# TigreGotico/phoonnx

Measured on AMD Instinct MI355X. Metric: audio samples/sec (22.05 kHz), batch-32 256-phoneme utterances, higher is better.
Workload: dtype f32 (f16x3 split: fp32 operands as two fp16 planes, three MFMA products, fp32 accumulate)

## Files before the change

### include/vitsmi.h

```cpp
#ifndef VITSMI_H
#define VITSMI_H

#include <stddef.h>
#include <stdint.h>

#ifdef __cplusplus
extern "C" {
#endif

typedef struct vits_handle vits_handle;

enum {
    VITS_OK = 0,
    VITS_E_IO = -1,
    VITS_E_FORMAT = -2,
    VITS_E_ARG = -3,
    VITS_E_DEVICE = -4,
    VITS_E_NOMEM = -5,
    VITS_E_RANGE = -6
};

#define VITS_MAX_DIMS 4


// ... 148 lines not shown
int vits_test_conv1d_sx(int device_id, const float *x, int B, int Cin, int T, const float *w, const float *bias,
                        int Cout, int K, int dil, int pad_l, int flags, float slope, float *out);
int vits_test_conv1d_sx_planar(int device_id, const float *x, int B, int Cin, int T, const float *w, const float *bias,
                               int Cout, int K, int dil, int flags, const int64_t *lens, const float *old, int row_split,
                               int pl_rows, float *out, float *planes_out);
long long vits_test_set_sx_small_max(long long wgs);
int vits_test_conv1d_sx_gate(int device_id, const float *x, int B, int Cin, int T, const float *w, const float *bias,
                             const float *bias_b, int Cout, int K, int dil, int flags, float *out);
int vits_test_conv_transpose1d_sx(int device_id, const float *x, int B, int Cin, int T, const float *w,
                                  const float *bias, int Cout, int K, int stride, float *out);
int vits_bench_conv1d_sx(int device_id, int B, int Cin, int Cout, int T, int K, int dil, int dbg, int iters,
                         float *ms_out);
int vits_test_conv_pair_sx(int device_id, const float *x, int B, int C, int T, const float *w1, const float *b1,
                           const float *w2, const float *b2, int K, int dil1, int dil2, int chain, float slope, float *out,
                           float *ms_out);
int vits_test_attention(int device_id, const float *qkv, int B, int C, int T, int n_heads, const float *rel_k,
                        const float *rel_v, int window, const int64_t *lens, float *out);
int vits_test_attention16(int device_id, const float *qkv, int B, int C, int T, int n_heads, const float *rel_k,
                          const float *rel_v, int window, const int64_t *lens, float *out, uint16_t *out_planes, int kernel,
                          int reps, float *ms_out);

int vits_test_resample(int device_id, const float *x, const int64_t *lens, int B, int S, int in_rate, int out_rate, float *y,
                       int64_t S_out);
int vits_test_resample_pieces(int device_id, const float *x, const int64_t *lens, int B, int S, int in_rate, int out_rate,
                              int piece_samples, float *y, int64_t S_out, int64_t *ranges, int max_ranges);

int vits_test_durations(int device_id, const float *logw, const int64_t *dur, const int64_t *lens, int B, int T, float length_scale,
                        const float *rows, const float *token_rate, float *w_ceil, int32_t *cum, int32_t *y_len);
int vits_test_expand_prior(int device_id, const float *m_logs, int B, int C, int T, const int32_t *cum, const int64_t *lens,
                           const int32_t *y_len, int F, const float *noise, int64_t noise_stride, int noise_frames,
// ... 12 lines not shown
```

### phoonnx_amd/_ffi.py

```python
import ctypes as C
import os

import numpy as np

_HERE = os.path.dirname(os.path.abspath(__file__))
_LIB = None

VITS_MAX_DIMS = 4


class VitsNoise(C.Structure):
    _fields_ = [("noise_dp", C.c_void_p), ("noise_z", C.c_void_p), ("noise_z_stride", C.c_int64),
                ("seed", C.c_uint64)]


class VitsOutput(C.Structure):
    _fields_ = [("data", C.POINTER(C.c_float)), ("dims", C.c_int64 * 4), ("y_lengths", C.POINTER(C.c_int64))]


class VitsStats(C.Structure):
    _fields_ = [("conv_flops", C.c_double), ("conv_bytes", C.c_double), ("dec_flops", C.c_double),
                ("dec_bytes", C.c_double), ("flow_flops", C.c_double), ("enc_flops", C.c_double),
                ("dp_flops", C.c_double), ("conv_ms", C.c_float), ("dec_ms", C.c_float), ("flow_ms", C.c_float),
                ("enc_ms", C.c_float), ("dp_ms", C.c_float), ("total_ms", C.c_float), ("conv_launches", C.c_int),
# ... 18 lines not shown

CHUNK_FN = C.CFUNCTYPE(C.c_int, C.c_void_p, C.POINTER(C.c_float), C.c_int, C.c_int64, C.c_int64, C.c_int64)

VITS_E_RANGE = -6


EXPORTS = [
    "vits_open", "vits_open_with_arena", "vits_open_host", "vits_open_layout", "vits_open_opts", "vits_close",
    "vits_run_chunked", "vits_run_vocoder_chunked", "vits_last_error", "vits_num_inputs",
    "vits_input_name", "vits_meta", "vits_hparam", "vits_arena_bytes", "vits_arena_host", "vits_arena_device",
    "vits_run", "vits_free_output", "vits_run_device", "vits_sync", "vits_last_y_lengths", "vits_last_pcm16", "vits_run_vocoder",
    "vits_tap",
    "vits_set_timing", "vits_set_tails", "vits_reserve", "vits_get_stats", "vits_stream", "vits_test_conv1d", "vits_test_conv_transpose1d",
    "vits_test_attention", "vits_test_attention16", "vits_bench_conv1d", "vits_test_conv1d_sx", "vits_test_conv1d_sx_planar", "vits_test_conv1d_sx_gate", "vits_test_set_sx_small_max",
    "vits_test_conv_transpose1d_sx",
    "vits_bench_conv1d_sx", "vits_test_conv_pair_sx", "vits_fetch_output", "vits_run_async", "vits_host_alloc", "vits_host_free",
    "vits_launch_records", "vits_run_async_rows", "vits_run_device_rows", "vits_run_chunked_rows",
    "vits_run_async_ctl", "vits_run_chunked_ctl", "vits_last_durations",
    "vits_set_output_rate", "vits_last_sample_counts", "vits_resample_plan", "vits_test_resample", "vits_test_resample_pieces",
    "vits_test_durations", "vits_test_expand_prior", "vits_test_fill_normal", "vits_test_fill_normal_rows", "vits_test_post_conv",
]


G2P_EXPORTS = ["g2p_open", "g2p_close", "g2p_last_error", "g2p_hparam", "g2p_num_outputs", "g2p_output_name", "g2p_bucket",
               "g2p_run", "g2p_generate", "g2p_generate_batch", "g2p_test_forced_steps", "g2p_test_linear", "g2p_test_step"]


def lib_path():
    return os.environ.get("VITSMI_LIB") or os.path.join(_HERE, "libvitsmi.so")


# ... 82 lines not shown
                                               C.c_int, vp]
    lib.vits_test_attention.argtypes = [C.c_int, vp, C.c_int, C.c_int, C.c_int, C.c_int, vp, vp, C.c_int, vp, vp]
    lib.vits_test_attention16.argtypes = [C.c_int, vp, C.c_int, C.c_int, C.c_int, C.c_int, vp, vp, C.c_int, vp, vp, vp,
                                          C.c_int, C.c_int, f32p]
    lib.vits_bench_conv1d.argtypes = [C.c_int] * 11 + [f32p]
    lib.vits_test_conv1d_sx.argtypes = lib.vits_test_conv1d.argtypes
    lib.vits_test_conv_transpose1d_sx.argtypes = lib.vits_test_conv_transpose1d.argtypes
    lib.vits_test_conv1d_sx_planar.argtypes = [C.c_int, vp, C.c_int, C.c_int, C.c_int, vp, vp, C.c_int, C.c_int, C.c_int, C.c_int,
                                               vp, vp, C.c_int, C.c_int, vp, vp]
    lib.vits_test_set_sx_small_max.argtypes = [C.c_longlong]
    lib.vits_test_set_sx_small_max.restype = C.c_longlong
    lib.vits_test_conv1d_sx_gate.argtypes = [C.c_int, vp, C.c_int, C.c_int, C.c_int, vp, vp, vp, C.c_int, C.c_int, C.c_int, C.c_int, vp]
    lib.vits_bench_conv1d_sx.argtypes = [C.c_int] * 9 + [f32p]
    lib.vits_test_conv_pair_sx.argtypes = [C.c_int, vp, C.c_int, C.c_int, C.c_int, vp, vp, vp, vp, C.c_int, C.c_int,
                                           C.c_int, C.c_int, C.c_float, vp, f32p]
    lib.g2p_open.argtypes = [C.c_char_p, C.c_int, C.POINTER(vp)]
    lib.g2p_close.argtypes = [vp]
    lib.g2p_close.restype = None
    lib.g2p_last_error.argtypes = [vp]
    lib.g2p_last_error.restype = C.c_char_p
    lib.g2p_hparam.argtypes = [vp, C.c_char_p, i64p]
    lib.g2p_num_outputs.argtypes = [vp]
    lib.g2p_output_name.argtypes = [vp, C.c_int]
    lib.g2p_output_name.restype = C.c_char_p
    lib.g2p_bucket.argtypes = [vp, C.c_int, C.c_int]
    lib.g2p_run.argtypes = [vp, vp, C.c_int, vp, vp, C.c_int, vp]
    lib.g2p_generate.argtypes = [vp, vp, C.c_int, C.c_int, C.c_int64, C.c_int64, vp, C.POINTER(C.c_int)]
    lib.g2p_generate_batch.argtypes = [vp, vp, vp, C.c_int, C.c_int, C.c_int64, C.c_int64, vp, vp]
    lib.g2p_test_forced_steps.argtypes = [vp, vp, vp, C.c_int, vp, C.c_int, vp]
    lib.g2p_test_linear.argtypes = [C.c_int, C.c_int, vp, vp, C.c_int, vp, C.c_int, C.c_int, vp, C.c_int64, C.c_int64, C.c_int, vp]
# ... 12 lines not shown
```

### phoonnx_amd/csrc/conv_sx_pair.hip.hpp

```cpp
#pragma once
#include <cstdlib>
#include "conv_geom.hpp"
#include "conv_sx_engine.hip.hpp"

namespace vitsmi {

struct SxPairArgs {
    const float *xr;
    float islope, mslope;
    int T;
    const u32x4 *wp1, *wp2;
    const float *bias1, *bias2;
    float wscale1, wscale2;
    float *out_raw;
    const float *zeros;
    int C, nchunks;
    int K1, dil1, pad1;
    int K2, dil2, pad2;
    int LW1;
    unsigned x_bytes;
    int LW2;
    unsigned y_chunk_bytes;
    int BNo, NT, B;
    int flags;
// ... 35 lines not shown
#ifndef SX_PAIR_WGS32
#define SX_PAIR_WGS32 3
#endif
#ifndef SX_PAIR_EARLY32
#define SX_PAIR_EARLY32 1
#endif
#ifndef SX_PAIR_ST_SC1
#define SX_PAIR_ST_SC1 0
#endif
#ifndef SX_PAIR_ONE_READ64
#define SX_PAIR_ONE_READ64 1
#endif
#ifndef SX_PAIR_ONE_READ32
#define SX_PAIR_ONE_READ32 1
#endif
template <int MW, int NW, int WM, int WN, int EPI, bool CHAIN, int NCH = 1>
__global__ __launch_bounds__(256, (NW == 2 && !SX_PAIR_EARLY_ACC && NCH == 1) ? SX_PAIR_WGS32 : 2) void conv_sx_pair_kernel(SxPairArgs a) {
    constexpr int BN = NW * WN * 32, NH = NW / 2;
    static_assert(NCH == 1 || (CHAIN && NW == 2 && (EPI & EPI_ACC) == 0), "fused chains: 32 channels, no external running sum");
    constexpr bool ONE_READ = NW == 4 ? SX_PAIR_ONE_READ64 != 0 : SX_PAIR_ONE_READ32 != 0;
    constexpr bool EARLY = ONE_READ || (NW == 2 && SX_PAIR_EARLY32);
    constexpr int DEPTH = NW == 2 ? SX_PAIR_DEPTH32 : SX_PAIR_DEPTH64;
    static_assert(DEPTH >= 2 && DEPTH <= 6, "wait_a covers up to five younger sets");
    constexpr bool ACC = (EPI & EPI_ACC) != 0 && SX_PAIR_EARLY_ACC;
    static_assert(!(ONE_READ && ACC), "the running sum is not pulled into the single-read prologue");
    static_assert(WM * WN == 4 && MW == 1 && BN == 256, "one block row per wave, 256 columns");
    constexpr int NPW = 2, STEPBYTES = WM * MW * NPW * 1024;
    constexpr int MAXCH = WM * 2;
    extern __shared__ __attribute__((aligned(16))) unsigned char lds_sx[];
    const int tid = threadIdx.x, lane = tid & 63;
    const int wave = __builtin_amdgcn_readfirstlane(tid >> 6);
    const int wm = wave / WN, wn = wave % WN;
    const int l31 = lane & 31, hi = lane >> 5;
    const int wg_xcd = blockIdx.x & 7, wg_seq = blockIdx.x >> 3;
    const int tile_nb = __builtin_amdgcn_readfirstlane(sx_xcd_tile(wg_seq, wg_xcd, a.xgs));
    if (tile_nb >= a.NT * a.B) return;
    const int b = tile_nb / a.NT, t0 = (tile_nb - b * a.NT) * a.BNo;
    const int t1 = t0 - a.pad2;
    const int T = a.T, LW = a.LW1;
    const int TV = __builtin_amdgcn_readfirstlane(sx_valid_cols(a.rag, b, T));
    if (t0 >= TV) return;
    const uint32_t lds0 = (uint32_t)(uintptr_t)lds_sx;
    const uint32_t XB = a.x_bytes;
    const char *wbase1 = reinterpret_cast<const char *>(a.wp1) + wm * (MW * NPW * 1024);
    const char *wbase2 = reinterpret_cast<const char *>(a.wp2) + wm * (MW * NPW * 1024);
    const float *xrb = a.xr + (int64_t)b * a.C * T;
    float pk = 0.f;

    struct ASet {
        u32x4 fa[2];
    };
    const uint32_t voff0 = (uint32_t)lane * 16u;
    auto load_a = [&](ASet &f, const char *wb, int step) {
// ... 29 lines not shown
        asm volatile("s_memtime %0\n\ts_waitcnt lgkmcnt(0)" : "=s"(t)::"memory");
        __builtin_amdgcn_sched_barrier(0);
        return t;
    };
    unsigned long long tp[8];
    tp[0] = stamp();
#endif
    if constexpr (NW == 2 && WM == 1 && NCH == 1 && SX_PAIR_SHARED_A != 0)
        for (int g = 0; g < 3; g++)
            if (g < ((a.nchunks * a.K1) >> 1)) {
                const int sub = wave >> 1, pl = wave & 1;
                lds_dma<16>(wbase1 + (int64_t)(2 * g + sub) * STEPBYTES + pl * 1024 + lane * 16,
                            reinterpret_cast<float *>(lds_sx + a.a_ring + (unsigned)((g * 2 + sub) * 2048 + pl * 1024)));
            }
    constexpr bool BIAS_LDS = NCH == 1;
    if constexpr (BIAS_LDS) {
        if (wave == 0) {
            constexpr int CC = WM * 32;
            const int k = lane - (lane >= CC / 4 ? CC / 4 : 0);
            const float *bp = lane < CC / 4 ? a.bias1 : a.bias2;
            const void *src = (bp && lane < CC / 2) ? static_cast<const void *>(bp + 4 * k) : static_cast<const void *>(a.zeros + 4 * (lane & 31));
            lds_dma<16>(src, reinterpret_cast<float *>(lds_sx + a.bias_off));
        }
    }
    auto bias_from_lds = [&](int conv, f32x4 (&bq)[4]) __attribute__((always_inline)) {
        u32x4 t4[4];
#pragma unroll
        for (int q = 0; q < 4; q++)
            asm volatile("ds_read_b128 %0, %1" : "=v"(t4[q]) : "v"(lds0 + a.bias_off + (uint32_t)(conv * (WM * 32) + wm * 32 + 8 * q + 4 * hi) * 4u) : "memory");
        asm volatile("s_waitcnt lgkmcnt(0)" ::: "memory");
        __builtin_amdgcn_sched_barrier(0);
#pragma unroll
        for (int q = 0; q < 4; q++) bq[q] = __builtin_bit_cast(f32x4, t4[q]);
    };
    constexpr int NXC = 3;
    if constexpr (ONE_READ) {
        constexpr int NXH = MAXCH, NG = 2 * MAXCH;
        const int HW = LW - 256, pad1 = a.pad1;
        const int nhc = HW * NG, nxh = (nhc + 255) >> 8;
        u32x4 hst[NXH][2];
        bool hin[NXH], hok[NXH];
        uint32_t hlds[NXH];
        const float *hp[NXH];
#pragma unroll
// ... 303 lines not shown
        for (int g = 0; g < NG; g++) {
            step(fa0, fa1, 2 * g, false);
            step(fa1, fa0, 2 * g + 1, true);
        }
    };

    struct ChainPar {
        const char *wb1, *wb2;
        const float *bias1, *bias2;
        float ws1, ws2;
        int K1, dil1, K2, dil2;
        uint32_t xoff, yoff;
    };
    auto chain_par = [&](int ci) {
        ChainPar c;
        if constexpr (NCH == 1) {
            c = ChainPar{wbase1, wbase2, a.bias1, a.bias2, a.wscale1, a.wscale2, a.K1, a.dil1, a.K2, a.dil2, 0u, 0u};
        } else {
            const auto &h = a.ch[ci];
            c = ChainPar{reinterpret_cast<const char *>(h.wp1) + wm * (MW * NPW * 1024),
                         reinterpret_cast<const char *>(h.wp2) + wm * (MW * NPW * 1024),
                         h.bias1, h.bias2, h.wscale1, h.wscale2, h.K1, h.dil1, h.K2, h.dil2, (uint32_t)h.xoff, (uint32_t)h.yoff};
        }
        return c;
    };
    static_assert(NCH == 1 || EARLY, "fused chains keep x in registers from the prologue on");
    const uint32_t ylds = NCH > 1 ? lds0 + (uint32_t)a.nchunks * XB : lds0;
    f32x4 xkeep[NCH > 1 ? NW / 2 : 1][2][4], tot[NCH > 1 ? NW / 2 : 1][2][4];
#if SX_PAIR_ALIAS
    ASet f1s[DEPTH + 1];
    ASet(&f2s)[DEPTH + 1] = f1s;
#else
    ASet f1s[DEPTH + 1], f2s[DEPTH + 1];
#endif
#pragma unroll 1
    for (int ci = 0; ci < NCH; ci++) {
    const ChainPar cp = chain_par(ci);
    if constexpr (NCH > 1) {
        if (ci > 0) {
#pragma unroll
            for (int rr = 0; rr < NW / 2; rr++)
#pragma unroll
                for (int j = 0; j < 2; j++)
#pragma unroll
                    for (int q = 0; q < 4; q++) pre[rr][j][q] = xkeep[rr][j][q];
            zero_acc();
        }
    }
    if constexpr (!SHA) load_a(f1s[0], cp.wb1, 0);
    if (ci == 0) {
        asm volatile("s_waitcnt lgkmcnt(0)" ::: "memory");
#if SX_PAIR_PROF
// ... 24 lines not shown
    if constexpr (SHA) sha_prefetch(cp.wb2, cp.K2);
    {
        const float wsc = cp.ws1, msl = a.mslope;
        const float *biasp = cp.bias1 ? cp.bias1 : a.zeros;
        const int b_on = cp.bias1 ? 1 : 0;
        const uint32_t YC = a.y_chunk_bytes, LW2 = (uint32_t)a.LW2;
        const int row0 = wm * 32;
        f32x4 bq[4];
        if constexpr (BIAS_LDS) bias_from_lds(0, bq);
        else {
#pragma unroll
            for (int q = 0; q < 4; q++) bq[q] = *reinterpret_cast<const f32x4 *>(biasp + (row0 + 8 * q + 4 * hi) * b_on);
        }
#pragma unroll
        for (int n = 0; n < NW; n++) {
            const int col = (wn * NW + n) * 32 + l31;
            const int t = t1 + col;
            const bool live = t >= 0 && t < TV;
#pragma unroll
            for (int q = 0; q < 4; q++) {
                float o[4];
#pragma unroll
                for (int e = 0; e < 4; e++) {
                    float v = __builtin_fmaf(acc[n][4 * q + e], wsc, bq[q][e]);
                    if constexpr (CHAIN) {
                        if constexpr (NCH > 1) {
                            if (ci == 0) xkeep[n / 2][n % 2][q][e] = pre[n / 2][n % 2][q][e];
                        }
                        v += pre[n / 2][n % 2][q][e];
                        pre[n / 2][n % 2][q][e] = v;
                    }
                    o[e] = live ? fmaxf(v, v * msl) : 0.f;
                }
                unsigned wa[2], wb[2];
                split2h_pair_pk(o[0], o[1], wa[0], wa[1], pk);
                split2h_pair_pk(o[2], o[3], wb[0], wb[1], pk);
                const int g = 4 * wm + q;
                const uint32_t cell = ylds + (uint32_t)(g >> 1) * YC + ((uint32_t)(g & 1) * LW2 + (uint32_t)(col + a.pad2)) * 16u + 8u * hi;
                asm volatile("ds_write_b64 %0, %1" ::"v"(cell), "v"(u32x2{wa[0], wb[0]}) : "memory");
                asm volatile("ds_write_b64 %0, %1" ::"v"(cell + 2u * LW2 * 16u), "v"(u32x2{wa[1], wb[1]}) : "memory");
            }
            asm volatile("" : "+v"(pk));
        }
    }
    zero_acc();
    asm volatile("s_waitcnt lgkmcnt(0)" ::: "memory");
    __builtin_amdgcn_s_barrier();
    __builtin_amdgcn_sched_barrier(0);
#if SX_PAIR_PROF
    tp[5] = stamp();
#endif

    if constexpr (SHA)
        run_conv_sha(f2s[0], f2s[1], cp.wb2, cp.K2, cp.dil2, ylds + (uint32_t)(hi * a.LW2 + wn * (NW * 32) + l31 + (int)cp.yoff) * 16u,
                     a.y_chunk_bytes, (uint32_t)(2 * a.LW2) * 16u);
    else
        run_conv(f2s, cp.wb2, cp.K2, cp.dil2, ylds + (uint32_t)(hi * a.LW2 + wn * (NW * 32) + l31 + (int)cp.yoff) * 16u,
                 a.y_chunk_bytes, (uint32_t)(2 * a.LW2) * 16u);
#if SX_PAIR_PROF
    tp[6] = stamp();
#endif
    if constexpr (!CHAIN && !EARLY) load_pre();

    {
        constexpr int flags = EPI;
        float *rawb = a.out_raw + (int64_t)b * a.C * T;
        const float wsc = cp.ws2, rdiv = a.div;
        const float *biasp = cp.bias2 ? cp.bias2 : a.zeros;
        const int b_on = cp.bias2 ? 1 : 0;
        const int row0 = wm * 32;
        f32x4 bq[4];
        if constexpr (BIAS_LDS) bias_from_lds(1, bq);
        else {
#pragma unroll
            for (int q = 0; q < 4; q++) bq[q] = *reinterpret_cast<const f32x4 *>(biasp + (row0 + 8 * q + 4 * hi) * b_on);
        }
        static_for<NW / 2>([&](auto R) {
            constexpr int rr = decltype(R)::value;
            f32x4 adl[2][4];
            if constexpr ((flags & EPI_ACC) != 0 && !(EARLY && ACC)) {
#pragma unroll
                for (int j = 0; j < 2; j++) {
                    const int t = t1 + (wn * NW + rr * 2 + j) * 32 + l31;
                    const int tl = t < 0 ? 0 : (t < T ? t : T - 1);
#pragma unroll
                    for (int q = 0; q < 4; q++)
                        adl[j][q] = *reinterpret_cast<const f32x4 *>(rawb + ((int64_t)((row0 >> 3) + q) * T + tl) * 8 + 4 * hi);
                }
            }
#pragma unroll
            for (int j = 0; j < 2; j++) {
                const int n = rr * 2 + j;
                const int col = (wn * NW + n) * 32 + l31;
                const int t = t1 + col;
                const bool kept = !(col < a.pad2 || col >= a.pad2 + a.BNo || t >= TV);
                if constexpr (NCH == 1) {
                    if (!kept) continue;
                }
#pragma unroll
                for (int q = 0; q < 4; q++) {
                    f32x4 v;
#pragma unroll
                    for (int e = 0; e < 4; e++) v[e] = __builtin_fmaf(acc[n][4 * q + e], wsc, bq[q][e]);
                    v += pre[rr][j][q];
                    if constexpr (NCH > 1) {
                        if (ci > 0) v += tot[rr][j][q];
                        tot[rr][j][q] = v;
                        if (ci < NCH - 1 || !kept) continue;
                    }
                    if constexpr ((flags & EPI_ACC) != 0) {
                        if constexpr (EARLY && ACC) v += ad[rr][j][q];
                        else v += adl[j][q];
                    }
                    if constexpr ((flags & EPI_DIV) != 0) {
#pragma unroll
                        for (int e = 0; e < 4; e++) v[e] = v[e] / rdiv;
                    }
#if SX_PAIR_ST_SC1
                    {
                        float *sp = rawb + ((int64_t)((row0 >> 3) + q) * T + t) * 8 + 4 * hi;
                        const f32x4 sv = v;
                        asm volatile("global_store_dwordx4 %0, %1, off sc1" ::"v"(sp), "v"(sv) : "memory");
                    }
#else
                    *reinterpret_cast<f32x4 *>(rawb + ((int64_t)((row0 >> 3) + q) * T + t) * 8 + 4 * hi) = v;
#endif
                }
            }
        });
    }
    }
#if SX_PAIR_PROF
    asm volatile("s_waitcnt vmcnt(0)" ::: "memory");
    tp[7] = stamp();
    if (a.prof && tid == 0) {
        for (int i = 0; i < 7; i++) atomicAdd(a.prof + i, tp[i + 1] - tp[i]);
        atomicAdd(a.prof + 7, 1ull);
    }
#endif
    if (a.peak) sx_publish_peak(a.peak, (int)blockIdx.x, pk);
}

template <int MW, int NW, int WM, int WN, int EPI, bool CHAIN, int NCH = 1>
inline hipError_t launch_conv_sx_pair_k(const SxPairArgs &a, dim3 grid, size_t lds, hipStream_t stream) {
    static std::atomic<uint64_t> attr_done{0};
    auto kern = conv_sx_pair_kernel<MW, NW, WM, WN, EPI, CHAIN, NCH>;
    if (hipError_t e = sx_allow_big_lds(reinterpret_cast<const void *>(kern), attr_done); e != hipSuccess) return e;
    if (g_launch_name_on)
        snprintf(g_launch_name, sizeof g_launch_name, "conv_sx_pair_kernel<%d, %d, %d, %d, %d, %s, %d>", MW, NW, WM, WN, EPI,
                 CHAIN ? "true" : "false", NCH);
    kern<<<grid, 256, lds, stream>>>(a);
    return hipGetLastError();
}

inline bool sx_pair_supported(int C, int cfg, int K1, int dil1, int K2, int dil2) {
    if (K1 < 3 || K2 < 3 || dil1 < 1 || dil2 < 1) return false;
    if (!((C == 64 && cfg == 1) || (C == 32 && cfg == 2))) return false;
    const int LW1 = 256 + (K1 - 1) * dil1;
    if (2 * LW1 > kSxRawStageCells) return false;
    const int halo2 = (K2 - 1) * dil2;
    static const int keep_min = [] {
        const char *e = std::getenv("VITSMI_PAIR_MIN_KEEP");
        return e ? std::atoi(e) : 160;
    }();
    if (halo2 % 2 || 256 - halo2 < keep_min) return false;
// ... 53 lines not shown
    }
    if (cfg == 1) {
        if (chain) {
            SX_PAIR_CASES(1, 4, 2, 2, true)
        }
        SX_PAIR_CASES(1, 4, 2, 2, false)
    }
    if (chain) {
        SX_PAIR_CASES(1, 2, 1, 4, true)
    }
    SX_PAIR_CASES(1, 2, 1, 4, false)
#undef SX_PAIR_CASES
}
#endif

struct SxMrfGeom {
    int pad1, pad2, LW1, LW2;
    size_t lds;
};
inline bool sx_mrf_geom(int C, int n, const int *K1, const int *dil1, const int *K2, const int *dil2, SxMrfGeom *g) {
    if (C != 32 || n < 2 || n > 3) return false;
    int p1 = 0, p2 = 0;
    for (int i = 0; i < n; i++) {
        if (K1[i] < 3 || K2[i] < 3 || !(K1[i] & 1) || !(K2[i] & 1) || dil1[i] < 1 || dil2[i] < 1) return false;
        const int a1 = (K1[i] - 1) / 2 * dil1[i], a2 = (K2[i] - 1) / 2 * dil2[i];
        p1 = a1 > p1 ? a1 : p1;
        p2 = a2 > p2 ? a2 : p2;
    }
    const int LW1 = 256 + 2 * p1;
    if (2 * LW1 > kSxRawStageCells) return false;
// ... 54 lines not shown
```

### phoonnx_amd/csrc/vitsmi.hip

```cpp
#include <climits>
#include <hip/hip_runtime.h>

#include <cmath>
#include <cstdarg>
#include <chrono>
#include <cstdio>
#include <cstring>
#include <mutex>
#include <string>
#include <vector>

#include "../../include/vitsmi.h"
#include "conv_geom.hpp"
#include "conv_sx_engine.hip.hpp"
#include "conv_sx_pair.hip.hpp"
#include "conv_sx_pair16.hip.hpp"
#include "attention16.hip.hpp"
#include "conv_sx_small.hip.hpp"
#include "kernels.hip.hpp"
#include "model.hpp"
#include "resample.hip.hpp"
#include "test_dev.hip.hpp"
#include "workspace.hpp"

// ... 652 lines not shown
                    fprintf(stderr, "pairprof row %d wgs %llu:", r, hrows[r * 8 + 7]);
                    for (int i = 0; i < 7; i++) fprintf(stderr, " %.0f", (double)hrows[r * 8 + i] / (double)hrows[r * 8 + 7]);
                    fprintf(stderr, "\n");
                }
            hipMemset(rows, 0, sizeof hrows);
        }
    }
#endif
    const bool ev = conv_event_begin(c);
    c.note(launch_conv_sx_pair(a, c1.cfg, c.B, c.st, chain));
    const double wf = c.work_frac();
    const double fl = 2.0 * (c1.macs_per_t + c2.macs_per_t) * (double)T * c.B * wf;
    const double by = 4.0 * c.B * ((double)(c1.Cin + c1.Cout) * T + (double)(c2.Cin + c2.Cout) * T) * wf;
    const ConvDesc *const members[] = {&c1, &c2};
    fused_launch_end(c, ev, members, 2, c1, T, fl, by);
}

bool sx_pair16_ok(const vits_handle *h, const ConvDesc &c1, const ConvDesc &c2) {
    static const bool off = [] {
        const char *e = std::getenv("VITSMI_PAIR16");
        return (e && e[0] == '0') || std::getenv("VITSMI_SX_NO_PAIR") != nullptr;
    }();
    if (off || c1.Cin != c1.Cout || c2.Cin != c2.Cout || c1.Cin != c2.Cin || c1.ups != 1 || c2.ups != 1) return false;
    if (c1.padL * 2 != (c1.K - 1) * c1.dil || c2.padL * 2 != (c2.K - 1) * c2.dil) return false;
    const bool h1 = c1.h1 && c2.h1, f3 = c1.f16 && c2.f16 && c1.s16 && c2.s16 && !c1.rawin && !c2.rawin;
    if (!h1 && !f3) return false;
    if (c1.cfg != c2.cfg || c1.cfg != (c1.Cin == 64 ? 1 : 2)) return false;
    (void)h;
    return sx_pair16_plan(c1.Cin, h1 ? 1 : 2, c1.K, c1.dil, c2.K, c2.dil, nullptr) != 0;
}
// ... 712 lines not shown
            auto step_out = [&](int q) {
                StepOut w{EPI_RES, rpl ? nullptr : ra[q & 1], fr ? nullptr : raa[q & 1]};
                if (q == rbk.n - 1) {
                    w.flags |= mrf_flags(j, nk);
                    w.raw = xs_raw;
                    w.pl = nullptr;
                    if (j == nk - 1 && !last_stage && !fr) {
                        w.pl = xs_pl;
                        w.flags |= SX_NO_RAW_STORE;
                    }
                }
                return w;
            };
            const float *cur = y_raw;
            const uint16_t *cura = y_pl;
            for (int q = 0; q < rbk.n; q++) {
                StepOut w = step_out(q);
                if (rbk.type1 && fr && sx_pair_ok(h, rbk.c1[q], rbk.c2[q])) {
                    conv_sx_pair(c, rbk.c1[q], rbk.c2[q], cur, T, w.raw, w.flags, (float)nk, S);
                } else if (!rbk.type1 && fr && q + 1 < rbk.n && sx_pair_ok(h, rbk.c1[q], rbk.c1[q + 1])) {
                    w = step_out(++q);
                    conv_sx_pair(c, rbk.c1[q - 1], rbk.c1[q], cur, T, w.raw, w.flags, (float)nk, S, true);
                } else {
                    const void *in = fr ? static_cast<const void *>(cur) : static_cast<const void *>(cura);
                    SxOpt res = rbk.type1 || rpl ? act : lrelu;
                    res.div = (float)nk;
                    if (rpl) {
                        res.res_pl = cura;
                        res.res_slope = S;
                    } else
// ... 1699 lines not shown
    a.C = C;
    a.K1 = d1.K; a.dil1 = d1.dil; a.pad1 = d1.padL;
    a.K2 = d2.K; a.dil2 = d2.dil; a.pad2 = d2.padL;
    a.div = 1.f;
    auto go = [&] { return launch_conv_sx_pair(a, d1.cfg, B, nullptr, chain != 0); };
    TCHECK(go());
    TCHECK(hipDeviceSynchronize());
    if (ms_out) TCHECK(time_launches(10, go, ms_out));
    sx_unblock_kernel<<<dim3((T + 255) / 256, C / 8, B), 256>>>(draw, nullptr, dout, C, T, 1);
    TCHECK(hipGetLastError());
    TCHECK(hipDeviceSynchronize());
    TCHECK(download(out, dout, n));
    return VITS_OK;
}

int vits_bench_conv1d_sx(int device_id, int B, int Cin, int Cout, int T, int K, int dil, int dbg, int iters,
                         float *ms_out) {
    if (int rc = test_dev(device_id)) return rc;
    std::vector<float> w((size_t)Cout * Cin * K), x((size_t)B * Cin * T);
    bench_fill(w, x);
    ConvDesc d;
    std::vector<float> arena;
    TestPack o = sx_test_pack((dbg & 64) ? SxPack::F16X1 : ((dbg & 128) ? SxPack::F16X2 : SxPack::BF16X3));
    o.sx.no_s16 = (dbg & (1 | 2 | 16 | 256)) != 0;
    std::string e = pack_test_conv(w.data(), nullptr, Cin, Cout, K, dil, dil * (K - 1) / 2, 3, &d, &arena, o);
    if (!e.empty()) return fail(nullptr, VITS_E_ARG, "%s", e.c_str());
    const size_t nx = x.size(), no = (size_t)B * Cout * T;
    DevBufs D;
    float *dA = D.up(arena.data(), arena.size());
    float *dx = D.up(x.data(), nx);
// ... 389 lines not shown
```

### phoonnx_amd/session.py

```python
import ctypes as C
import time
from dataclasses import dataclass
from typing import Dict, List, Optional, Sequence

import numpy as np

from . import _ffi


class SessionError(RuntimeError):
    """Raised for every failure of the engine (onnxruntime raises its own
    InvalidArgument/RuntimeException at voice.py:374; callers there do not catch either)."""


class RangeError(SessionError):
    """VITS_E_RANGE: the f16x3 generator arithmetic met an activation beyond the range of its fp16 operand planes
    (|x| > 65504) or a non-finite value.  The engine reports this instead of returning clamped audio; `MiSession`
    (range_fallback=True, the default) then reopens the voice with the bf16x6 arithmetic (fp32 range) and repeats the
    call, so user code only sees this when the fallback is switched off or impossible (borrowed weight arena)."""


class _PinnedPool:

    def __init__(self, keep_bytes=2 << 30):
# ... 1077 lines not shown
        raise ValueError("both convs are C -> C with the same kernel size")
    b1 = None if b1 is None else np.ascontiguousarray(b1, np.float32)
    b2 = None if b2 is None else np.ascontiguousarray(b2, np.float32)
    out = np.empty_like(x)
    ms = C.c_float(0.0)
    rc = lib.vits_test_conv_pair_sx(device_id, _ffi.ptr(x), B, Cc, T, _ffi.ptr(w1), _ffi.ptr(b1), _ffi.ptr(w2),
                                    _ffi.ptr(b2), K, dil1, dil2,
                                    (1 if chain else 0) | ({"pair": 0, "pair16": 1, "pair16_f16": 2}[kernel] << 1) | (8 if from_plane else 0),
                                    float(slope), _ffi.ptr(out),
                                    C.byref(ms) if timed else None)
    if rc != 0:
        raise SessionError(_ffi.last_error(None))
    return (out, float(ms.value)) if timed else out


def bench_conv1d_sx(B, Cin, Cout, T, K, dil=1, dbg=0, iters=20, device_id=0):
    lib = _ffi.load()
    res = np.zeros(8, np.float32)
    rc = lib.vits_bench_conv1d_sx(device_id, B, Cin, Cout, T, K, dil, dbg, iters,
                                  res.ctypes.data_as(_ffi.C.POINTER(_ffi.C.c_float)))
    if rc != 0:
        raise SessionError(_ffi.last_error(None))
    if dbg & 16:
        return float(res[0]), int(res[1]), [float(v) for v in res[3:8]] + [float(res[2])]
    return float(res[0]), int(res[1])


def test_conv_transpose1d(x, w, bias, stride, device_id=0, sx=False):
    lib = _ffi.load()
    x = np.ascontiguousarray(x, np.float32)
# ... 205 lines not shown
```

Measured before the change: 142.1 million.

## Fuse all steps of a ResBlock1 into one conv-pair kernel launch

Adds an NSTEP template mode to the paired-conv kernel so the 2-3 dilated conv pairs of one HiFi-GAN ResBlock1 run inside a single launch. Intermediate residual sums stay in registers and in LDS as fp16 planes instead of round-tripping through global memory between steps. Each tile computes shrinking halo margins and keeps only the central columns. This removes per-step launches and activation reads and writes, at the cost of redundant halo compute and larger LDS per workgroup, which may lower occupancy. A test and benchmark entry point is added as well.

Measured after the change: 143.3 million (median of 6 runs). Within noise of the previous version (+0.9%).

```diff
diff --git a/include/vitsmi.h b/include/vitsmi.h
--- a/include/vitsmi.h
+++ b/include/vitsmi.h
@@ -186,6 +186,8 @@
 int vits_test_conv_pair_sx(int device_id, const float *x, int B, int C, int T, const float *w1, const float *b1,
                            const float *w2, const float *b2, int K, int dil1, int dil2, int chain, float slope, float *out,
                            float *ms_out);
+int vits_test_resblock1_sx(int device_id, const float *x, int B, int C, int T, const float *ws, const float *bs, int K, int nstep,
+                           const int *dils, float slope, const float *acc, float div, float *out, float *ms_out);
 int vits_test_attention(int device_id, const float *qkv, int B, int C, int T, int n_heads, const float *rel_k,
                         const float *rel_v, int window, const int64_t *lens, float *out);
 int vits_test_attention16(int device_id, const float *qkv, int B, int C, int T, int n_heads, const float *rel_k,
diff --git a/phoonnx_amd/_ffi.py b/phoonnx_amd/_ffi.py
--- a/phoonnx_amd/_ffi.py
+++ b/phoonnx_amd/_ffi.py
@@ -56,7 +56,7 @@
     "vits_set_timing", "vits_set_tails", "vits_reserve", "vits_get_stats", "vits_stream", "vits_test_conv1d", "vits_test_conv_transpose1d",
     "vits_test_attention", "vits_test_attention16", "vits_bench_conv1d", "vits_test_conv1d_sx", "vits_test_conv1d_sx_planar", "vits_test_conv1d_sx_gate", "vits_test_set_sx_small_max",
     "vits_test_conv_transpose1d_sx",
-    "vits_bench_conv1d_sx", "vits_test_conv_pair_sx", "vits_fetch_output", "vits_run_async", "vits_host_alloc", "vits_host_free",
+    "vits_bench_conv1d_sx", "vits_test_conv_pair_sx", "vits_test_resblock1_sx", "vits_fetch_output", "vits_run_async", "vits_host_alloc", "vits_host_free",
     "vits_launch_records", "vits_run_async_rows", "vits_run_device_rows", "vits_run_chunked_rows",
     "vits_run_async_ctl", "vits_run_chunked_ctl", "vits_last_durations",
     "vits_set_output_rate", "vits_last_sample_counts", "vits_resample_plan", "vits_test_resample", "vits_test_resample_pieces",
@@ -169,6 +169,8 @@
     lib.vits_bench_conv1d_sx.argtypes = [C.c_int] * 9 + [f32p]
     lib.vits_test_conv_pair_sx.argtypes = [C.c_int, vp, C.c_int, C.c_int, C.c_int, vp, vp, vp, vp, C.c_int, C.c_int,
                                            C.c_int, C.c_int, C.c_float, vp, f32p]
+    lib.vits_test_resblock1_sx.argtypes = [C.c_int, vp, C.c_int, C.c_int, C.c_int, vp, vp, C.c_int, C.c_int, vp, C.c_float, vp,
+                                           C.c_float, vp, f32p]
     lib.g2p_open.argtypes = [C.c_char_p, C.c_int, C.POINTER(vp)]
     lib.g2p_close.argtypes = [vp]
     lib.g2p_close.restype = None
diff --git a/phoonnx_amd/csrc/conv_sx_pair.hip.hpp b/phoonnx_amd/csrc/conv_sx_pair.hip.hpp
--- a/phoonnx_amd/csrc/conv_sx_pair.hip.hpp
+++ b/phoonnx_amd/csrc/conv_sx_pair.hip.hpp
@@ -73,10 +73,11 @@
 #ifndef SX_PAIR_ONE_READ32
 #define SX_PAIR_ONE_READ32 1
 #endif
-template <int MW, int NW, int WM, int WN, int EPI, bool CHAIN, int NCH = 1>
+template <int MW, int NW, int WM, int WN, int EPI, bool CHAIN, int NCH = 1, int NSTEP = 1>
 __global__ __launch_bounds__(256, (NW == 2 && !SX_PAIR_EARLY_ACC && NCH == 1) ? SX_PAIR_WGS32 : 2) void conv_sx_pair_kernel(SxPairArgs a) {
     constexpr int BN = NW * WN * 32, NH = NW / 2;
     static_assert(NCH == 1 || (CHAIN && NW == 2 && (EPI & EPI_ACC) == 0), "fused chains: 32 channels, no external running sum");
+    static_assert(NSTEP == 1 || (!CHAIN && NCH == 1 && NSTEP <= 3), "sequential steps: the steps of one ResBlock1, parameters in a.ch[]");
     constexpr bool ONE_READ = NW == 4 ? SX_PAIR_ONE_READ64 != 0 : SX_PAIR_ONE_READ32 != 0;
     constexpr bool EARLY = ONE_READ || (NW == 2 && SX_PAIR_EARLY32);
     constexpr int DEPTH = NW == 2 ? SX_PAIR_DEPTH32 : SX_PAIR_DEPTH64;
@@ -95,7 +96,11 @@
     const int tile_nb = __builtin_amdgcn_readfirstlane(sx_xcd_tile(wg_seq, wg_xcd, a.xgs));
     if (tile_nb >= a.NT * a.B) return;
     const int b = tile_nb / a.NT, t0 = (tile_nb - b * a.NT) * a.BNo;
-    const int t1 = t0 - a.pad2;
+    auto keep0 = [&]() {
+        if constexpr (NSTEP > 1) return (256 - a.BNo) >> 1;
+        else return a.pad2;
+    };
+    const int t1 = t0 - keep0();
     const int T = a.T, LW = a.LW1;
     const int TV = __builtin_amdgcn_readfirstlane(sx_valid_cols(a.rag, b, T));
     if (t0 >= TV) return;
@@ -155,20 +160,24 @@
                             reinterpret_cast<float *>(lds_sx + a.a_ring + (unsigned)((g * 2 + sub) * 2048 + pl * 1024)));
             }
     constexpr bool BIAS_LDS = NCH == 1;
+    uint32_t bias_step = 0;
     if constexpr (BIAS_LDS) {
-        if (wave == 0) {
+        bool mine = wave == 0;
+        if constexpr (NSTEP > 1) mine = wave < NSTEP;
+        if (mine) {
             constexpr int CC = WM * 32;
             const int k = lane - (lane >= CC / 4 ? CC / 4 : 0);
             const float *bp = lane < CC / 4 ? a.bias1 : a.bias2;
+            if constexpr (NSTEP > 1) bp = lane < CC / 4 ? a.ch[wave].bias1 : a.ch[wave].bias2;
             const void *src = (bp && lane < CC / 2) ? static_cast<const void *>(bp + 4 * k) : static_cast<const void *>(a.zeros + 4 * (lane & 31));
-            lds_dma<16>(src, reinterpret_cast<float *>(lds_sx + a.bias_off));
+            lds_dma<16>(src, reinterpret_cast<float *>(lds_sx + a.bias_off + (NSTEP > 1 ? wave * 1024 : 0)));
         }
     }
     auto bias_from_lds = [&](int conv, f32x4 (&bq)[4]) __attribute__((always_inline)) {
         u32x4 t4[4];
 #pragma unroll
         for (int q = 0; q < 4; q++)
-            asm volatile("ds_read_b128 %0, %1" : "=v"(t4[q]) : "v"(lds0 + a.bias_off + (uint32_t)(conv * (WM * 32) + wm * 32 + 8 * q + 4 * hi) * 4u) : "memory");
+            asm volatile("ds_read_b128 %0, %1" : "=v"(t4[q]) : "v"(lds0 + a.bias_off + bias_step + (uint32_t)(conv * (WM * 32) + wm * 32 + 8 * q + 4 * hi) * 4u) : "memory");
         asm volatile("s_waitcnt lgkmcnt(0)" ::: "memory");
         __builtin_amdgcn_sched_barrier(0);
 #pragma unroll
@@ -502,7 +511,7 @@
     };
     auto chain_par = [&](int ci) {
         ChainPar c;
-        if constexpr (NCH == 1) {
+        if constexpr (NCH == 1 && NSTEP == 1) {
             c = ChainPar{wbase1, wbase2, a.bias1, a.bias2, a.wscale1, a.wscale2, a.K1, a.dil1, a.K2, a.dil2, 0u, 0u};
         } else {
             const auto &h = a.ch[ci];
@@ -521,9 +530,22 @@
 #else
     ASet f1s[DEPTH + 1], f2s[DEPTH + 1];
 #endif
-#pragma unroll 1
-    for (int ci = 0; ci < NCH; ci++) {
-    const ChainPar cp = chain_par(ci);
+    constexpr int NIT = NSTEP > 1 ? NSTEP : NCH;
+    int marg = 0;
+    constexpr int UNROLL = NSTEP > 1 ? NSTEP : 1;
+#pragma unroll UNROLL
+    for (int ci = 0; ci < NIT; ci++) {
+    ChainPar cp = chain_par(ci);
+    int marg1 = 0;
+    if constexpr (NSTEP > 1) {
+        asm volatile("" : "+s"(cp.wb1), "+s"(cp.wb2), "+s"(cp.ws1), "+s"(cp.ws2));
+        asm volatile("" : "+s"(cp.K1), "+s"(cp.dil1), "+s"(cp.K2), "+s"(cp.dil2), "+s"(cp.xoff), "+s"(cp.yoff));
+        __builtin_amdgcn_sched_barrier(0);
+        bias_step = (uint32_t)ci * 1024u;
+        marg1 = marg + (ci > 0 ? a.pad1 - (int)cp.xoff : 0);
+    }
+    int l31s = l31, his = hi;
+    if constexpr (NSTEP > 1) asm volatile("" : "+v"(l31s), "+v"(his));
     if constexpr (NCH > 1) {
         if (ci > 0) {
 #pragma unroll
@@ -578,9 +600,10 @@
         }
 #pragma unroll
         for (int n = 0; n < NW; n++) {
-            const int col = (wn * NW + n) * 32 + l31;
+            const int col = (wn * NW + n) * 32 + l31s;
             const int t = t1 + col;
-            const bool live = t >= 0 && t < TV;
+            bool live = t >= 0 && t < TV;
+            if constexpr (NSTEP > 1) live = live && col >= marg1 && col < 256 - marg1;
 #pragma unroll
             for (int q = 0; q < 4; q++) {
                 float o[4];
@@ -600,7 +623,7 @@
                 split2h_pair_pk(o[0], o[1], wa[0], wa[1], pk);
                 split2h_pair_pk(o[2], o[3], wb[0], wb[1], pk);
                 const int g = 4 * wm + q;
-                const uint32_t cell = ylds + (uint32_t)(g >> 1) * YC + ((uint32_t)(g & 1) * LW2 + (uint32_t)(col + a.pad2)) * 16u + 8u * hi;
+                const uint32_t cell = ylds + (uint32_t)(g >> 1) * YC + ((uint32_t)(g & 1) * LW2 + (uint32_t)(col + a.pad2)) * 16u + 8u * his;
                 asm volatile("ds_write_b64 %0, %1" ::"v"(cell), "v"(u32x2{wa[0], wb[0]}) : "memory");
                 asm volatile("ds_write_b64 %0, %1" ::"v"(cell + 2u * LW2 * 16u), "v"(u32x2{wa[1], wb[1]}) : "memory");
             }
@@ -625,6 +648,52 @@
     tp[6] = stamp();
 #endif
     if constexpr (!CHAIN && !EARLY) load_pre();
+
+    if constexpr (NSTEP > 1) {
+        if (ci < NSTEP - 1) {
+            marg = marg1 + a.pad2;
+            const float wsc = cp.ws2, isl = a.islope;
+            const int pad1 = a.pad1;
+            f32x4 bq[4];
+            bias_from_lds(1, bq);
+            __builtin_amdgcn_s_barrier();
+            __builtin_amdgcn_sched_barrier(0);
+            asm volatile("" : "+v"(l31s), "+v"(his));
+#pragma unroll
+            for (int n = 0; n < NW; n++) {
+                const int col = (wn * NW + n) * 32 + l31s;
+                const int t = t1 + col;
+                const bool ok = t >= 0 && t < TV && col >= marg && col < 256 - marg;
+#pragma unroll
+                for (int q = 0; q < 4; q++) {
+                    f32x4 r;
+#pragma unroll
+                    for (int e = 0; e < 4; e++) r[e] = __builtin_fmaf(acc[n][4 * q + e], wsc, bq[q][e]);
+                    r += pre[n / 2][n % 2][q];
+                    pre[n / 2][n % 2][q] = r;
+                    float v[4];
+#pragma unroll
+                    for (int e = 0; e < 4; e++) {
+                        const float x = ok ? r[e] : 0.f;
+                        v[e] = fmaxf(x, x * isl);
+                    }
+                    unsigned wa[2], wb[2];
+                    split2h_pair_pk(v[0], v[1], wa[0], wa[1], pk);
+                    split2h_pair_pk(v[2], v[3], wb[0], wb[1], pk);
+                    const int g = 4 * wm + q;
+                    const uint32_t cell = lds0 + (uint32_t)(g >> 1) * XB + (uint32_t)((g & 1) * LW + pad1 + col) * 16u + 8u * his;
+                    asm volatile("ds_write_b64 %0, %1" ::"v"(cell), "v"(u32x2{wa[0], wb[0]}) : "memory");
+                    asm volatile("ds_write_b64 %0, %1" ::"v"(cell + (uint32_t)(2 * LW) * 16u), "v"(u32x2{wa[1], wb[1]}) : "memory");
+                }
+                asm volatile("" : "+v"(pk));
+            }
+            zero_acc();
+            asm volatile("s_waitcnt lgkmcnt(0)" ::: "memory");
+            __builtin_amdgcn_s_barrier();
+            __builtin_amdgcn_sched_barrier(0);
+            continue;
+        }
+    }
 
     {
         constexpr int flags = EPI;
@@ -637,7 +706,7 @@
         if constexpr (BIAS_LDS) bias_from_lds(1, bq);
         else {
 #pragma unroll
-            for (int q = 0; q < 4; q++) bq[q] = *reinterpret_cast<const f32x4 *>(biasp + (row0 + 8 * q + 4 * hi) * b_on);
+            for (int q = 0; q < 4; q++) bq[q] = *reinterpret_cast<const f32x4 *>(biasp + (row0 + 8 * q + 4 * his) * b_on);
         }
         static_for<NW / 2>([&](auto R) {
             constexpr int rr = decltype(R)::value;
@@ -645,19 +714,19 @@
             if constexpr ((flags & EPI_ACC) != 0 && !(EARLY && ACC)) {
 #pragma unroll
                 for (int j = 0; j < 2; j++) {
-                    const int t = t1 + (wn * NW + rr * 2 + j) * 32 + l31;
+                    const int t = t1 + (wn * NW + rr * 2 + j) * 32 + l31s;
                     const int tl = t < 0 ? 0 : (t < T ? t : T - 1);
 #pragma unroll
                     for (int q = 0; q < 4; q++)
-                        adl[j][q] = *reinterpret_cast<const f32x4 *>(rawb + ((int64_t)((row0 >> 3) + q) * T + tl) * 8 + 4 * hi);
+                        adl[j][q] = *reinterpret_cast<const f32x4 *>(rawb + ((int64_t)((row0 >> 3) + q) * T + tl) * 8 + 4 * his);
                 }
             }
 #pragma unroll
             for (int j = 0; j < 2; j++) {
                 const int n = rr * 2 + j;
-                const int col = (wn * NW + n) * 32 + l31;
+                const int col = (wn * NW + n) * 32 + l31s;
                 const int t = t1 + col;
-                const bool kept = !(col < a.pad2 || col >= a.pad2 + a.BNo || t >= TV);
+                const bool kept = !(col < keep0() || col >= keep0() + a.BNo || t >= TV);
                 if constexpr (NCH == 1) {
                     if (!kept) continue;
                 }
@@ -682,12 +751,12 @@
                     }
 #if SX_PAIR_ST_SC1
                     {
-                        float *sp = rawb + ((int64_t)((row0 >> 3) + q) * T + t) * 8 + 4 * hi;
+                        float *sp = rawb + ((int64_t)((row0 >> 3) + q) * T + t) * 8 + 4 * his;
                         const f32x4 sv = v;
                         asm volatile("global_store_dwordx4 %0, %1, off sc1" ::"v"(sp), "v"(sv) : "memory");
                     }
 #else
-                    *reinterpret_cast<f32x4 *>(rawb + ((int64_t)((row0 >> 3) + q) * T + t) * 8 + 4 * hi) = v;
+                    *reinterpret_cast<f32x4 *>(rawb + ((int64_t)((row0 >> 3) + q) * T + t) * 8 + 4 * his) = v;
 #endif
                 }
             }
@@ -705,14 +774,14 @@
     if (a.peak) sx_publish_peak(a.peak, (int)blockIdx.x, pk);
 }
 
-template <int MW, int NW, int WM, int WN, int EPI, bool CHAIN, int NCH = 1>
+template <int MW, int NW, int WM, int WN, int EPI, bool CHAIN, int NCH = 1, int NSTEP = 1>
 inline hipError_t launch_conv_sx_pair_k(const SxPairArgs &a, dim3 grid, size_t lds, hipStream_t stream) {
     static std::atomic<uint64_t> attr_done{0};
-    auto kern = conv_sx_pair_kernel<MW, NW, WM, WN, EPI, CHAIN, NCH>;
+    auto kern = conv_sx_pair_kernel<MW, NW, WM, WN, EPI, CHAIN, NCH, NSTEP>;
     if (hipError_t e = sx_allow_big_lds(reinterpret_cast<const void *>(kern), attr_done); e != hipSuccess) return e;
     if (g_launch_name_on)
-        snprintf(g_launch_name, sizeof g_launch_name, "conv_sx_pair_kernel<%d, %d, %d, %d, %d, %s, %d>", MW, NW, WM, WN, EPI,
-                 CHAIN ? "true" : "false", NCH);
+        snprintf(g_launch_name, sizeof g_launch_name, "conv_sx_pair_kernel<%d, %d, %d, %d, %d, %s, %d, %d>", MW, NW, WM, WN, EPI,
+                 CHAIN ? "true" : "false", NCH, NSTEP);
     kern<<<grid, 256, lds, stream>>>(a);
     return hipGetLastError();
 }
@@ -796,6 +865,100 @@
 }
 #endif
 
+struct SxRb1Geom {
+    int pad1, pad2, LW1, LW2, BNo;
+    size_t lds;
+};
+inline bool sx_rb1_supported(int C, int cfg, int K, const int *dils, int n, SxRb1Geom *g = nullptr) {
+    if (n < 2 || n > 3 || K < 3 || !(K & 1)) return false;
+    const int pad2 = (K - 1) / 2;
+    int pmax = 0, lose = n * pad2;
+    for (int s = 0; s < n; s++) {
+        if (!sx_pair_supported(C, cfg, K, dils[s], K, 1)) return false;
+        const int p = pad2 * dils[s];
+        pmax = p > pmax ? p : pmax;
+        if (s > 0) lose += p;
+    }
+    const int LW1 = 256 + 2 * pmax, LW2 = (256 + pad2 + 7) / 8 * 8, BNo = 256 - 2 * lose;
+    if (2 * LW1 > kSxRawStageCells) return false;
+    static const int keep32 = [] {
+        const char *e = std::getenv("VITSMI_RB1_MIN_KEEP");
+        return e ? std::atoi(e) : 234;
+    }();
+    static const int keep64 = [] {
+        const char *e = std::getenv("VITSMI_RB1_MIN_KEEP64");
+        return e ? std::atoi(e) : 234;
+    }();
+    if (BNo < (C == 64 ? keep64 : keep32) || BNo < 64) return false;
+    const size_t lds_x = (size_t)(C / 16) * 4 * LW1 * 16, lds_y = (size_t)(C / 16) * 4 * LW2 * 16 + (size_t)pad2 * 16;
+    const size_t lds = ((lds_x > lds_y ? lds_x : lds_y) + 15) / 16 * 16 + (size_t)n * 1024;
+    if (lds > (size_t)(C == 32 ? 40 * 1024 : kLdsTwoPerCu)) return false;
+    if (g) *g = SxRb1Geom{pmax, pad2, LW1, LW2, BNo, lds};
+    return true;
+}
+
+hipError_t launch_conv_sx_rb1(SxPairArgs a, int cfg, int B, hipStream_t stream);
+#ifdef VITSMI_IMPL_PAIR
+hipError_t launch_conv_sx_rb1(SxPairArgs a, int cfg, int B, hipStream_t stream) {
+    const int n = a.nchain;
+    if (n < 2 || n > 3) return hipErrorInvalidValue;
+    int dils[3];
+    for (int s = 0; s < n; s++) {
+        const auto &h = a.ch[s];
+        if (h.K1 != a.ch[0].K1 || h.K2 != h.K1 || h.dil2 != 1) return hipErrorInvalidValue;
+        dils[s] = h.dil1;
+    }
+    SxRb1Geom g;
+    if (!sx_rb1_supported(a.C, cfg, a.ch[0].K1, dils, n, &g)) return hipErrorInvalidValue;
+    for (int s = 0; s < n; s++) {
+        a.ch[s].xoff = g.pad1 - g.pad2 * dils[s];
+        a.ch[s].yoff = 0;
+        if (a.ch[s].wscale1 == 0.f) a.ch[s].wscale1 = 1.f;
+        if (a.ch[s].wscale2 == 0.f) a.ch[s].wscale2 = 1.f;
+    }
+    a.pad1 = g.pad1;
+    a.pad2 = g.pad2;
+    a.LW1 = g.LW1;
+    a.x_bytes = (unsigned)((size_t)4 * a.LW1 * 16);
+    a.LW2 = g.LW2;
+    a.y_chunk_bytes = (unsigned)(4 * a.LW2 * 16);
+    a.BNo = g.BNo;
+    a.NT = (a.T + a.BNo - 1) / a.BNo;
+    a.B = B;
+    a.nchunks = a.C / 16;
+    if (a.islope == 0.f) a.islope = 1.f;
+    if (a.mslope == 0.f) a.mslope = 1.f;
+    if ((long long)a.T * 64 + 64 >= (1ll << 32)) return hipErrorInvalidValue;
+    a.bias_off = (unsigned)(g.lds - (size_t)n * 1024);
+    const long long nb = (long long)a.NT * B;
+    if (nb == 0) return hipSuccess;
+    a.xgs = a.NT >= (2 << sx_xcd_group_shift()) ? sx_xcd_group_shift() : 0;
+    const long long per_round = 8ll << a.xgs;
+    const long long wgs = (nb + per_round - 1) / per_round * per_round;
+    if (wgs >= (1ll << 31)) return hipErrorInvalidValue;
+    dim3 grid((unsigned)wgs, 1, 1);
+    const int epi = a.flags & (EPI_ACC | EPI_DIV);
+    if ((epi & EPI_DIV) && !(epi & EPI_ACC)) return hipErrorInvalidValue;
+#define SX_RB1_CASES(NW, WM, WN, NS)                                                                                  \
+    switch (epi) {                                                                                                    \
+        case 0: return launch_conv_sx_pair_k<1, NW, WM, WN, 0, false, 1, NS>(a, grid, g.lds, stream);                 \
+        case EPI_ACC: return launch_conv_sx_pair_k<1, NW, WM, WN, EPI_ACC, false, 1, NS>(a, grid, g.lds, stream);     \
+        default: return launch_conv_sx_pair_k<1, NW, WM, WN, EPI_ACC | EPI_DIV, false, 1, NS>(a, grid, g.lds, stream); \
+    }
+    if (cfg == 1) {
+        if (n == 2) {
+            SX_RB1_CASES(4, 2, 2, 2)
+        }
+        SX_RB1_CASES(4, 2, 2, 3)
+    }
+    if (n == 2) {
+        SX_RB1_CASES(2, 1, 4, 2)
+    }
+    SX_RB1_CASES(2, 1, 4, 3)
+#undef SX_RB1_CASES
+}
+#endif
+
 struct SxMrfGeom {
     int pad1, pad2, LW1, LW2;
     size_t lds;
diff --git a/phoonnx_amd/csrc/vitsmi.hip b/phoonnx_amd/csrc/vitsmi.hip
--- a/phoonnx_amd/csrc/vitsmi.hip
+++ b/phoonnx_amd/csrc/vitsmi.hip
@@ -690,6 +690,60 @@
     const double by = 4.0 * c.B * ((double)(c1.Cin + c1.Cout) * T + (double)(c2.Cin + c2.Cout) * T) * wf;
     const ConvDesc *const members[] = {&c1, &c2};
     fused_launch_end(c, ev, members, 2, c1, T, fl, by);
+}
+
+bool sx_rb1_ok(const vits_handle *h, const ResBlockDesc &rb) {
+    static const bool off = std::getenv("VITSMI_SX_NO_RB1") != nullptr;
+    if (off || !rb.type1 || rb.n < 2 || rb.n > 3) return false;
+    int dils[3];
+    for (int q = 0; q < rb.n; q++) {
+        const ConvDesc &c1 = rb.c1[q], &c2 = rb.c2[q];
+        if (!sx_pair_ok(h, c1, c2) || c1.padL * 2 != (c1.K - 1) * c1.dil) return false;
+        if (c1.K != rb.c1[0].K || c2.K != c1.K || c2.dil != 1 || c1.cfg != rb.c1[0].cfg) return false;
+        dils[q] = c1.dil;
+    }
+    return sx_rb1_supported(rb.c1[0].Cin, rb.c1[0].cfg, rb.c1[0].K, dils, rb.n);
+}
+
+void conv_sx_rb1(Ctx &c, const ResBlockDesc &rb, const float *x, int T, float *out, int flags, float div, float slope) {
+    SxPairArgs a{};
+    a.xr = x;
+    a.islope = slope;
+    a.mslope = slope;
+    a.T = T;
+    a.out_raw = out;
+    a.zeros = c.P(c.m.zeros_off);
+    a.C = rb.c1[0].Cin;
+    a.flags = flags & (EPI_ACC | EPI_DIV);
+    a.div = div;
+    a.nchain = rb.n;
+    double macs = 0, bytes = 0;
+    const ConvDesc *members[6];
+    for (int q = 0; q < rb.n; q++) {
+        const ConvDesc &c1 = rb.c1[q], &c2 = rb.c2[q];
+        members[2 * q] = &c1;
+        members[2 * q + 1] = &c2;
+        auto &ch = a.ch[q];
+        ch.wp1 = reinterpret_cast<const u32x4 *>(c.P(c1.w_off));
+        ch.wp2 = reinterpret_cast<const u32x4 *>(c.P(c2.w_off));
+        ch.bias1 = c.P(c1.b_off);
+        ch.bias2 = c.P(c2.b_off);
+        ch.wscale1 = c1.wscale;
+        ch.wscale2 = c2.wscale;
+        ch.K1 = c1.K;
+        ch.dil1 = c1.dil;
+        ch.K2 = c2.K;
+        ch.dil2 = c2.dil;
+        macs += c1.macs_per_t + c2.macs_per_t;
+        bytes += 4.0 * ((double)(c1.Cin + c1.Cout) + (double)(c2.Cin + c2.Cout));
+    }
+    a.rag = c.rag_at(T);
+    a.peak = range_slots(c.h, true);
+    macs *= c.work_frac();
+    bytes *= c.work_frac();
+    const bool ev = conv_event_begin(c);
+    c.note(launch_conv_sx_rb1(a, rb.c1[0].cfg, c.B, c.st));
+    fused_launch_end(c, ev, members, 2 * rb.n, rb.c1[0], T, 2.0 * macs * (double)T * c.B, bytes * T * c.B);
 }
 
 bool sx_pair16_ok(const vits_handle *h, const ConvDesc &c1, const ConvDesc &c2) {
@@ -1432,6 +1486,11 @@
             };
             const float *cur = y_raw;
             const uint16_t *cura = y_pl;
+            if (fr && sx_rb1_ok(h, rbk)) {
+                const StepOut w = step_out(rbk.n - 1);
+                conv_sx_rb1(c, rbk, cur, T, w.raw, w.flags, (float)nk, S);
+                continue;
+            }
             for (int q = 0; q < rbk.n; q++) {
                 StepOut w = step_out(q);
                 if (rbk.type1 && fr && sx_pair_ok(h, rbk.c1[q], rbk.c2[q])) {
@@ -3161,6 +3220,97 @@
     return VITS_OK;
 }
 
+int vits_test_resblock1_sx(int device_id, const float *x, int B, int C, int T, const float *ws, const float *bs, int K, int nstep,
+                           const int *dils, float slope, const float *acc, float div, float *out, float *ms_out) {
+    if (int rc = test_dev(device_id)) return rc;
+    if (nstep < 2 || nstep > 3 || !dils || K < 1 || C < 1) return fail(nullptr, VITS_E_ARG, "a ResBlock1 of 2 or 3 steps");
+    ConvDesc d[3][2];
+    std::vector<float> arena;
+    TestPack o = sx_test_pack(SxPack::F16X2);
+    const size_t wn = (size_t)C * C * K;
+    for (int q = 0; q < nstep; q++)
+        for (int i = 0; i < 2; i++) {
+            const int dil = i == 0 ? dils[q] : 1;
+            if (dil < 1) return fail(nullptr, VITS_E_ARG, "dilation %d", dil);
+            std::string e = pack_test_conv(ws + (size_t)(2 * q + i) * wn, bs ? bs + (size_t)(2 * q + i) * C : nullptr, C, C, K, dil,
+                                           dil * (K - 1) / 2, 3, &d[q][i], &arena, o);
+            if (!e.empty()) return fail(nullptr, VITS_E_ARG, "%s", e.c_str());
+        }
+    bool ok = true;
+    for (int q = 0; q < nstep; q++)
+        ok = ok && d[q][0].rawin && d[q][1].rawin && d[q][0].cfg == d[0][0].cfg && d[q][1].cfg == d[0][0].cfg;
+    if (!ok || !sx_rb1_supported(C, d[0][0].cfg, K, dils, nstep))
+        return fail(nullptr, VITS_E_ARG, "this ResBlock1 cannot run as one launch (C %d, kernel %d, %d steps)", C, K, nstep);
+    const int cfg = d[0][0].cfg;
+    const size_t n = (size_t)B * C * T;
+    DevBufs D;
+    float *dA = D.up(arena.data(), arena.size());
+    float *dx = D.up(x, n, 16);
+    float *dacc = acc ? D.up(acc, n, 16) : nullptr;
+    float *dxr = D.alloc<float>(n, 16);
+    float *draw = D.fill<float>(n, 0, 16);
+    float *dmid[2] = {ms_out ? D.alloc<float>(n, 16) : nullptr, ms_out ? D.alloc<float>(n, 16) : nullptr};
+    float *dout = D.alloc<float>(n, 16);
+    TCHECK(D.err);
+    sx_block_kernel<<<dim3((T + 255) / 256, C / 8, B), 256>>>(dx, (int64_t)C * T, T, nullptr, dxr, C, T);
+    if (dacc) sx_block_kernel<<<dim3((T + 255) / 256, C / 8, B), 256>>>(dacc, (int64_t)C * T, T, nullptr, draw, C, T);
+    SxPairArgs a{};
+    a.xr = dxr;
+    a.islope = a.mslope = slope;
+    a.T = T;
+    a.out_raw = draw;
+    a.zeros = dA;
+    a.C = C;
+    a.flags = (acc ? EPI_ACC : 0) | (acc && div != 1.f ? EPI_DIV : 0);
+    a.div = div;
+    a.nchain = nstep;
+    SxPairArgs ap[3];
+    for (int q = 0; q < nstep; q++) {
+        auto &ch = a.ch[q];
+        const ConvDesc &c1 = d[q][0], &c2 = d[q][1];
+        ch.wp1 = reinterpret_cast<const u32x4 *>(dA + c1.w_off);
+        ch.wp2 = reinterpret_cast<const u32x4 *>(dA + c2.w_off);
+        ch.bias1 = c1.b_off >= 0 ? dA + c1.b_off : nullptr;
+        ch.bias2 = c2.b_off >= 0 ? dA + c2.b_off : nullptr;
+        ch.wscale1 = c1.wscale;
+        ch.wscale2 = c2.wscale;
+        ch.K1 = c1.K; ch.dil1 = c1.dil; ch.K2 = c2.K; ch.dil2 = c2.dil;
+        SxPairArgs &p = ap[q];
+        p = SxPairArgs{};
+        p.xr = q == 0 ? dxr : dmid[(q - 1) & 1];
+        p.islope = p.mslope = slope;
+        p.T = T;
+        p.wp1 = ch.wp1; p.wp2 = ch.wp2; p.bias1 = ch.bias1; p.bias2 = ch.bias2;
+        p.wscale1 = ch.wscale1; p.wscale2 = ch.wscale2;
+        p.out_raw = q == nstep - 1 ? dout : dmid[q & 1];
+        p.zeros = dA;
+        p.C = C;
+        p.K1 = c1.K; p.dil1 = c1.dil; p.pad1 = c1.padL;
+        p.K2 = c2.K; p.dil2 = c2.dil; p.pad2 = c2.padL;
+        p.div = 1.f;
+    }
+    auto go = [&] { return launch_conv_sx_rb1(a, cfg, B, nullptr); };
+    TCHECK(go());
+    TCHECK(hipDeviceSynchronize());
+    sx_unblock_kernel<<<dim3((T + 255) / 256, C / 8, B), 256>>>(draw, nullptr, dout, C, T, 1);
+    TCHECK(hipGetLastError());
+    TCHECK(hipDeviceSynchronize());
+    TCHECK(download(out, dout, n));
+    if (ms_out) {
+        auto go3 = [&] {
+            hipError_t e = hipSuccess;
+            for (int q = 0; q < nstep && e == hipSuccess; q++) e = launch_conv_sx_pair(ap[q], cfg, B, nullptr, false);
+            return e;
+        };
+        a.flags = 0;
+        TCHECK(go3());
+        TCHECK(hipDeviceSynchronize());
+        TCHECK(time_launches(10, go, ms_out));
+        TCHECK(time_launches(10, go3, ms_out + 1));
+    }
+    return VITS_OK;
+}
+
 int vits_bench_conv1d_sx(int device_id, int B, int Cin, int Cout, int T, int K, int dil, int dbg, int iters,
                          float *ms_out) {
     if (int rc = test_dev(device_id)) return rc;
diff --git a/phoonnx_amd/session.py b/phoonnx_amd/session.py
--- a/phoonnx_amd/session.py
+++ b/phoonnx_amd/session.py
@@ -1115,6 +1115,33 @@
     return (out, float(ms.value)) if timed else out
 
 
+def test_resblock1_sx(x, ws, bs, dils, slope=0.1, acc=None, div=1.0, timed=False, device_id=0):
+    lib = _ffi.load()
+    x = np.ascontiguousarray(x, np.float32)
+    ws = np.ascontiguousarray(ws, np.float32)
+    B, Cc, T = x.shape
+    n = len(dils)
+    if ws.ndim != 5 or ws.shape[:4] != (n, 2, Cc, Cc):
+        raise ValueError("ws is [steps][2][C][C][K]")
+    K = ws.shape[4]
+    bs = None if bs is None else np.ascontiguousarray(bs, np.float32)
+    if bs is not None and bs.shape != (n, 2, Cc):
+        raise ValueError("bs is [steps][2][C]")
+    acc = None if acc is None else np.ascontiguousarray(acc, np.float32)
+    if acc is not None and acc.shape != x.shape:
+        raise ValueError("acc has the shape of x")
+    if acc is None and float(div) != 1.0:
+        raise ValueError("a divisor needs a running sum")
+    d = np.ascontiguousarray(dils, np.int32)
+    out = np.empty_like(x)
+    ms = (C.c_float * 2)(0.0, 0.0)
+    rc = lib.vits_test_resblock1_sx(device_id, _ffi.ptr(x), B, Cc, T, _ffi.ptr(ws), _ffi.ptr(bs), K, n, _ffi.ptr(d), float(slope),
+                                    _ffi.ptr(acc), float(div), _ffi.ptr(out), ms if timed else None)
+    if rc != 0:
+        raise SessionError(_ffi.last_error(None))
+    return (out, float(ms[0]), float(ms[1])) if timed else out
+
+
 def bench_conv1d_sx(B, Cin, Cout, T, K, dil=1, dbg=0, iters=20, device_id=0):
     lib = _ffi.load()
     res = np.zeros(8, np.float32)
```
